# QuantEcon/dynamic_factor_models

Hardware: NVIDIA H100
Metric: EM iters/sec (N=200,r=8,T=500) (higher is better)
Workload: dtype f64

## Files before the change

dynamic_factor_models_b200/csrc/dfm_api.cu:

```cuda
#include "../../include/dfm_b200.h"
#include "dfm_common.cuh"
#include "dfm_kernels_np.cuh"
#include "dfm_kernels_em.cuh"
#include "dfm_kernels_emb.cuh"
#include "dfm_kernels_fused.cuh"
#include "dfm_kernels_fused2.cuh"
#include "dfm_kernels_als_masked.cuh"
#include "dfm_kernels_rep.cuh"
#include "dfm_kernels_inst.cuh"
#include <algorithm>
#include <new>
#include <thread>
#include <vector>
#ifndef DFM_EMU
#include <dlfcn.h>
#endif

#ifdef DFM_EMU
typedef int cudaError_t;
enum { cudaSuccess = 0 };
enum cudaMemcpyKind { cudaMemcpyHostToDevice, cudaMemcpyDeviceToHost, cudaMemcpyDeviceToDevice };
static inline cudaError_t cudaMalloc(void** p, size_t n) { *p = malloc(n ? n : 1); return *p ? 0 : 2; }
static inline cudaError_t cudaFree(void* p) { free(p); return 0; }
static inline cudaError_t cudaMemcpyAsync(void* d, const void* s, size_t n, cudaMemcpyKind, cudaStream_t) { memcpy(d, s, n); return 0; }
// ... 164 lines not shown
    cudaOccupancyMaxActiveBlocksPerMultiprocessor(&occ, k_em_fused<RT>, 128, smem);
    if (occ < 1) occ = 1;
    grid = std::min(B, h->nsm * occ);
  } else grid = std::min(B, h->nsm * 8);
#endif
  double* scr = arena->get<double>((size_t)std::min(B, h->nsm * 8) * T * FUSED_SCR(RT));
  if (dry) return DFM_OK;
  FusedArgs a2 = fa; a2.scratch = scr;
  L(k_em_fused<RT>, grid, 1, 128, smem, a2);
  (void)scratch_out;
  return DFM_OK;
}

struct EmbPlan {
  bool on; int ncb, ntE, nsE, nper, ntM, tsM, tper;
  double *Bpart, *qpart, *Spart, *sxxpart, *Cpart; int* counters;
  size_t smE, smM;
};
static EmbPlan emb_plan(int T, int N, int r, int batch, int nsm) {
  EmbPlan e{};
  e.on = r <= 32 && !getenv("DFM_NO_EMB");
  if (!e.on) return e;
  e.ncb = (r + 7) / 8;
  const int target = 2 * nsm;
  e.ntE = (T + EMB_TILE - 1) / EMB_TILE;
  int want = (target + e.ntE * batch - 1) / (e.ntE * batch);
  int ns = std::max((N + EMB_MAXSPLIT - 1) / EMB_MAXSPLIT, std::min(want, (N + 31) / 32));
  e.nper = (((N + ns - 1) / ns) + 3) & ~3;
  e.nsE = (N + e.nper - 1) / e.nper;
  e.ntM = (N + EMB_TILE - 1) / EMB_TILE;
  want = (target + e.ntM * batch - 1) / (e.ntM * batch);
  int ts = std::max(1, std::min(want, (T + 31) / 32));
  e.tper = (((T + ts - 1) / ts) + 3) & ~3;
  e.tsM = (T + e.tper - 1) / e.tper;
  if ((long long)e.nsE * batch > 65535 || (long long)e.tsM * batch > 65535) { e.on = false; return e; }
  e.smE = ((size_t)e.ncb * 8 * emb_pad(e.nper) + e.nper + 48) * 8;
  e.smM = ((size_t)2 * r * r + (size_t)2 * EMB_TILE * (r + 1) + 96) * 8;
  return e;
}
template <int NCB>
static int emb_launch_E(dfm_handle* h, const EmbPlan& e, const double* x, const double* dW, const double* dR, const double* dlogR, int T, int N,
                        int r, int batch, double* dBt, double* dqt, double* dslr, int* dnt, EmState* st) {
  DFM_SET_SMEM(k_emb_contract<NCB>, e.smE);
  L(k_emb_contract<NCB>, e.ntE, e.nsE * batch, 256, e.smE, x, dW, dR, dlogR, T, N, r, e.nsE, e.nper, batch, e.Bpart, e.qpart, e.counters,
    dBt, dqt, dslr, dnt, st);
  return DFM_OK;
}
template <int NCB>
static int emb_launch_M(dfm_handle* h, const EmbPlan& e, const double* x, const double* dFs, const double* dSff, int T, int N, int r, int batch,
                        double* dL, double* dR, double* dW, double* dlogR, EmState* st) {
  DFM_SET_SMEM(k_emb_mstep<NCB>, e.smM);
  L(k_emb_mstep<NCB>, e.ntM, e.tsM * batch, 256, e.smM, x, dFs, dSff, T, N, r, e.tsM, e.tper, batch, e.Spart, e.sxxpart,
    e.counters + (size_t)batch * e.ntE, dL, dR, dW, dlogR, e.Cpart, st);
  return DFM_OK;
}

static int run_em_general(dfm_handle* h, const double* x, const dfm_em_opts* o, double* dL, double* dR, double* dA, double* dQ, double* dP0,
                          double* dAn, double* dQn, double* dW, double* dlogR, double* dC, double* dBt, double* dqt, double* dslr, int* dnt,
                          double* dCt, double* dzp, double* dzf, double* dPp, double* dPf, double* dFs, double* dPsF, double* dSff, double* dll,
                          EmState* st, int* dit, int* dstat, int* active, int ntC, int nblkC, size_t smFS, int stgT, int want_psf, double* dxch, const EmbPlan& emb) {
  int T = o->T, N = o->N, r = o->r, p = o->p, batch = o->batch, mi = o->max_iter;
  int np = r * (r + 1) / 2;
  int* dsrc = dnt + (size_t)batch * T;
  int ntFS = (batch <= 2 * h->nsm) ? 512 : 256;
  if (getenv("DFM_FS_THREADS")) ntFS = atoi(getenv("DFM_FS_THREADS"));
  int ncl = 1;
  if (dxch && !getenv("DFM_NO_CLUSTER")) { if (batch * 8 <= h->nsm) ncl = 8; else if (batch * 4 <= h->nsm) ncl = 4; else if (batch * 2 <= h->nsm) ncl = 2; }
  if (getenv("DFM_CLUSTER")) ncl = std::max(1, std::min(8, atoi(getenv("DFM_CLUSTER"))));
  L(k_em_state_init, batch, 1, 1, 0, st);
  L(k_em_scan, N, batch, 64, 0, x, dL, T, N, r, st);
  L(k_em_prep, batch, 1, 128, 0, dL, dR, N, r, p, dW, dlogR, dC, dA, dAn, dQ, dQn, st, mi, 0, emb.on ? 1 : 0);
  if (emb.on) {
    L(k_emb_cinit, emb.ntM, batch, 256, 0, dL, dW, N, r, emb.Cpart, st);
    L(k_emb_close, batch, 1, 256, 0, N, r, p, emb.ntM, emb.Cpart, dC, dA, dAn, dQ, dQn, st, mi, 0);
  }
  int n_missing = batch;
  if (emb.on) {
    L(k_em_count_missing, 1, 1, 128, 48 * 8, st, batch, active);
    CK(cudaMemcpyAsync(&n_missing, active, sizeof(int), cudaMemcpyDeviceToHost, h->stream));
    CK(cudaStreamSynchronize(h->stream));
    CK(cudaMemsetAsync(emb.counters, 0, sizeof(int) * (size_t)batch * (emb.ntE + emb.ntM), h->stream));
  }
  const bool any_missing = n_missing > 0, any_bal = emb.on ? (n_missing < batch) : true;
  const int emb_on = emb.on ? 1 : 0;
  int h_active = batch;
  for (int it = 0; it < mi && h_active > 0; ++it) {
    if (any_missing) L(k_em_contract, nblkC, batch, ntC, ((size_t)(np + r) * ntC + 8) * 8, x, dL, dW, dR, dlogR, dC, T, N, r, dBt, dqt, dslr, dnt, dCt, st);
    if (any_bal) {
      if (!emb.on) L(k_em_contract_bal, (T + 31) / 32, batch, 256, 8 * 32 * 3 * 8, x, dW, dR, dlogR, T, N, r, dBt, dqt, dslr, dnt, st);
      else switch (emb.ncb) {
        case 1: emb_launch_E<1>(h, emb, x, dW, dR, dlogR, T, N, r, batch, dBt, dqt, dslr, dnt, st); break;
        case 2: emb_launch_E<2>(h, emb, x, dW, dR, dlogR, T, N, r, batch, dBt, dqt, dslr, dnt, st); break;
        case 3: emb_launch_E<3>(h, emb, x, dW, dR, dlogR, T, N, r, batch, dBt, dqt, dslr, dnt, st); break;
        default: emb_launch_E<4>(h, emb, x, dW, dR, dlogR, T, N, r, batch, dBt, dqt, dslr, dnt, st); break;
      }
    }
#ifndef DFM_EMU
    if (ncl > 1) {
      PROF_BEGIN("k_em_filter_smooth");
      cudaLaunchConfig_t cfg = {};
      cfg.gridDim = dim3((unsigned)(batch * ncl)); cfg.blockDim = dim3((unsigned)ntFS); cfg.dynamicSmemBytes = smFS; cfg.stream = h->stream;
      cudaLaunchAttribute at[1];
      at[0].id = cudaLaunchAttributeClusterDimension; at[0].val.clusterDim.x = (unsigned)ncl; at[0].val.clusterDim.y = 1; at[0].val.clusterDim.z = 1;
      cfg.attrs = at; cfg.numAttrs = 1;
      cudaError_t ce = cudaLaunchKernelEx(&cfg, k_em_filter_smooth, (const double*)dA, (const double*)dQ, (const double*)dP0, (const double*)dC,
                            (const double*)dBt, (const double*)dqt, (const double*)dslr, (const int*)dnt, (const double*)dCt, T, r, p, dzp, dzf,
                            dPp, dPf, dFs, dPsF, dSff, dAn, dQn, dll, mi, o->tol, st, dsrc, stgT, want_psf, dxch);
      PROF_END(); h->launches++;
      if (ce != cudaSuccess) {
        (void)cudaGetLastError();
        ncl = 1;
        L(k_em_filter_smooth, batch, 1, ntFS, smFS, dA, dQ, dP0, dC, dBt, dqt, dslr, dnt, dCt, T, r, p, dzp, dzf, dPp, dPf,
          dFs, dPsF, dSff, dAn, dQn, dll, mi, o->tol, st, dsrc, stgT, want_psf, (double*)nullptr);
      }
    } else
#endif
    L(k_em_filter_smooth, batch, 1, ntFS, smFS, dA, dQ, dP0, dC, dBt, dqt, dslr, dnt, dCt, T, r, p, dzp, dzf, dPp, dPf,
      dFs, dPsF, dSff, dAn, dQn, dll, mi, o->tol, st, dsrc, stgT, want_psf, (double*)nullptr);
    if (any_missing || !emb.on) L(k_em_mstep_series, N, batch, 64, (size_t)(2 * np + r + 8) * 8, x, dFs, dPsF, dSff, T, N, r, dL, dR, st, emb_on);
    if (any_bal && emb.on) {
      switch (emb.ncb) {
        case 1: emb_launch_M<1>(h, emb, x, dFs, dSff, T, N, r, batch, dL, dR, dW, dlogR, st); break;
        case 2: emb_launch_M<2>(h, emb, x, dFs, dSff, T, N, r, batch, dL, dR, dW, dlogR, st); break;
        case 3: emb_launch_M<3>(h, emb, x, dFs, dSff, T, N, r, batch, dL, dR, dW, dlogR, st); break;
        default: emb_launch_M<4>(h, emb, x, dFs, dSff, T, N, r, batch, dL, dR, dW, dlogR, st); break;
      }
      L(k_emb_close, batch, 1, 256, 0, N, r, p, emb.ntM, emb.Cpart, dC, dA, dAn, dQ, dQn, st, mi, 1);
    }
    if (any_missing || !emb.on) L(k_em_prep, batch, 1, 128, 0, dL, dR, N, r, p, dW, dlogR, dC, dA, dAn, dQ, dQn, st, mi, 1, emb_on);
    if (o->tol > 0 && ((it & 3) == 3)) {
      L(k_em_count_active, 1, 1, 128, 48 * 8, st, batch, active);
      CK(cudaMemcpyAsync(&h_active, active, sizeof(int), cudaMemcpyDeviceToHost, h->stream));
      CK(cudaStreamSynchronize(h->stream));
    }
  }
  L(k_em_collect, batch, 1, 1, 0, st, dit, dstat);
  return DFM_OK;
}

template <int RT>
static int launch_fused2(dfm_handle* h, const FusedArgs& fa, int B, int T, int N, Arena* arena, bool dry) {
  size_t smem = fused2_smem_doubles<RT>(T, N) * 8;
  int grid = std::min(B, h->nsm * 8);
  double* scr = arena->get<double>((size_t)std::min(B, h->nsm * 8) * T * FUSED_SCR(RT));
  if (dry) return DFM_OK;
#ifndef DFM_EMU
  DFM_SET_SMEM(k_em_fused2<RT>, smem);
  int occ = 1;
  cudaOccupancyMaxActiveBlocksPerMultiprocessor(&occ, k_em_fused2<RT>, 256, smem);
  if (occ < 1) occ = 1;
  grid = std::min(B, h->nsm * occ);
#endif
  FusedArgs a2 = fa; a2.scratch = scr;
  CUtensorMap tm; int rc_ = make_panel_tmap(h, fa.X, T, (long long)B * N, &tm); if (rc_) return rc_;
  L(k_em_fused2<RT>, grid, 1, 256, smem, a2, tm);
  return DFM_OK;
}

template <int RT>
static int launch_als_fused2(dfm_handle* h, const AlsFusedArgs& fa, int B, int T, int N) {
  size_t smem = als_fused2_smem_doubles<RT>(T, N) * 8;
  int grid = std::min(B, h->nsm * 8);
#ifndef DFM_EMU
  DFM_SET_SMEM(k_als_fused2<RT>, smem);
  int occ = 1;
  cudaOccupancyMaxActiveBlocksPerMultiprocessor(&occ, k_als_fused2<RT>, 256, smem);
  if (occ < 1) occ = 1;
  grid = std::min(B, h->nsm * occ);
#endif
  CUtensorMap tm; int rc_ = make_panel_tmap(h, fa.Xs, T, (long long)B * N, &tm); if (rc_) return rc_;
  L(k_als_fused2<RT>, grid, 1, 256, smem, fa, tm);
  return DFM_OK;
}
template <int RT>
static int launch_als_masked(dfm_handle* h, const AlsMaskedArgs& fa, int B, int T, int N) {
  size_t smem = als_masked_smem_doubles<RT>(T, N) * 8;
  int grid = std::min(B, h->nsm * 2);
#ifndef DFM_EMU
  DFM_SET_SMEM(k_als_masked<RT>, smem);
  int occ = 1;
  cudaOccupancyMaxActiveBlocksPerMultiprocessor(&occ, k_als_masked<RT>, 256, smem);
  if (occ < 1) occ = 1;
  grid = std::min(B, h->nsm * occ);
#endif
  L(k_als_masked<RT>, grid, 1, 256, smem, fa);
  return DFM_OK;
}
static bool als_masked_shape_ok(int T, int N, int r) {
  if (r < 1 || r > 8) return false;
  return ((size_t)r * (T | 1) + (size_t)r * (N | 1) + 5 * (size_t)r * r + 48) * 8 <= 100 * 1024;
}
static bool als_fused2_shape_ok(int T, int N, int r) {
  if (r < 1 || r > 8 || T < 4 || (T & 1)) return false;
  return ((size_t)FZ * pad4mod16(T) + (size_t)r * pad4mod16(N) + (size_t)N + 4 * (size_t)r * r + 2 * r + 48 +
          2 * F2_NCW * 72 + (size_t)F2_S * F2_STG + 32) * 8 <= 113 * 1024;
}

template <int RT> static int fused2_capacity_t(int nsm, int T, int N) {
#ifdef DFM_EMU
  (void)nsm; (void)T; (void)N; return 4;
#else
  size_t smem = fused2_smem_doubles<RT>(T, N) * 8;
  DFM_SET_SMEM(k_em_fused2<RT>, smem);
  int occ = 1;
  cudaOccupancyMaxActiveBlocksPerMultiprocessor(&occ, k_em_fused2<RT>, 256, smem);
  return nsm * (occ < 1 ? 1 : occ);
#endif
}
static int fused2_capacity(int nsm, int r, int T, int N) {
  switch (r) {
#define DFM_CASEC(RT) case RT: return fused2_capacity_t<RT>(nsm, T, N);
    DFM_CASEC(1) DFM_CASEC(2) DFM_CASEC(3) DFM_CASEC(4) DFM_CASEC(5) DFM_CASEC(6) DFM_CASEC(7) DFM_CASEC(8)
#undef DFM_CASEC
  }
  return 1;
}

static bool fused2_shape_ok(int T, int N, int r, int p) {
  if (p != 1 || r < 1 || r > 8 || T < 4 || (T & 1)) return false;
  size_t need = ((size_t)FZ * pad4mod16(T) + (size_t)r * pad4mod16(N) + 3 * (size_t)N + 30 * (size_t)r * r + 2 * (size_t)r +
                 std::max((size_t)97 * r + (size_t)r * r, (size_t)2 * F2_NCW * 72) + (size_t)F2_S * F2_STG + 106) * 8;
  return need <= 113 * 1024;
}

static bool fused_shape_ok(int T, int N, int r, int p) {
  if (p != 1 || r < 1 || r > 8 || T < 3) return false;
  return ((size_t)FZ * pad4mod16(T) + (size_t)r * pad4mod16(N) + 3 * (size_t)N + 31 * (size_t)r * r + 66 * (size_t)r + 128) * 8 <= kMaxSmem;
}

extern "C" {

int dfm_version(void) { return DFM_VERSION; }

const char* dfm_status_string(int s) {
  switch (s) {
    case DFM_OK: return "ok";
    case DFM_ERR_ARG: return "bad argument";
    case DFM_ERR_TOO_FEW_OBS: return "too few observations";
    case DFM_ERR_NOT_PD: return "matrix not positive definite";
    case DFM_ERR_NOT_CONVERGED: return "not converged (max_iter reached)";
    case DFM_ERR_CUDA: return "CUDA error / no device";
    case DFM_ERR_UNSUPPORTED: return "unsupported problem size";
    case DFM_ERR_NCCL: return "NCCL error";
  }
  return "unknown";
}

static void handle_teardown(dfm_handle* h) {
  if (!h) return;
  if (h->stream) cudaStreamSynchronize(h->stream);
  if (h->ws) cudaFree(h->ws);
  if (h->own_stream && h->stream) cudaStreamDestroy(h->stream);
#ifndef DFM_EMU
  if (h->copy_stream) { cudaStreamSynchronize(h->copy_stream); cudaStreamDestroy(h->copy_stream); }
  if (h->pinned_one) cudaFreeHost(h->pinned_one);
  if (h->d2h_stream) { cudaStreamSynchronize(h->d2h_stream); cudaStreamDestroy(h->d2h_stream); }
  if (h->done_host) cudaFreeHost(h->done_host);
  if (h->prof) for (auto& r : *h->prof) { cudaEventDestroy(r.e0); cudaEventDestroy(r.e1); }
#endif
  delete h->prof;
  delete h;
}

int dfm_create_on_stream(int device, void* cuda_stream, dfm_handle** out) {
  if (!out) return DFM_ERR_ARG;
  *out = nullptr;
  int ndev = 0;
  if (cudaGetDeviceCount(&ndev) != cudaSuccess || ndev <= 0 || device < 0 || device >= ndev) return DFM_ERR_CUDA;
  if (cudaSetDevice(device) != cudaSuccess) return DFM_ERR_CUDA;
  dfm_handle* h = new (std::nothrow) dfm_handle();
  if (!h) return DFM_ERR_CUDA;
  h->device = device; h->ws = nullptr; h->ws_bytes = 0; h->launches = 0; h->err[0] = 0;
  h->nsm = 132;
  h->profile = 0; h->prof = new std::vector<ProfRec>();
  h->stream = nullptr; h->own_stream = false;
  h->copy_stream = nullptr; h->pinned_one = nullptr; h->d2h_stream = nullptr; h->done_host = nullptr; h->done_dev = nullptr; h->done_cap = 0;
#ifndef DFM_EMU
  if (cudaDeviceGetAttribute(&h->nsm, cudaDevAttrMultiProcessorCount, device) != cudaSuccess || h->nsm <= 0) { handle_teardown(h); return DFM_ERR_CUDA; }
  if (cudaStreamCreateWithFlags(&h->copy_stream, cudaStreamNonBlocking) != cudaSuccess) { h->copy_stream = nullptr; handle_teardown(h); return DFM_ERR_CUDA; }
  if (cudaStreamCreateWithFlags(&h->d2h_stream, cudaStreamNonBlocking) != cudaSuccess) { h->d2h_stream = nullptr; handle_teardown(h); return DFM_ERR_CUDA; }
  if (cudaHostAlloc((void**)&h->pinned_one, sizeof(int), cudaHostAllocDefault) != cudaSuccess) { h->pinned_one = nullptr; handle_teardown(h); return DFM_ERR_CUDA; }
  *h->pinned_one = 1;
#endif
  if (cuda_stream) { h->stream = (cudaStream_t)cuda_stream; h->own_stream = false; }
  else { if (cudaStreamCreate(&h->stream) != cudaSuccess) { h->stream = nullptr; handle_teardown(h); return DFM_ERR_CUDA; } h->own_stream = true; }
  DFM_SET_SMEM(k_em_filter_smooth, kMaxSmem); DFM_SET_SMEM(k_als_factor, kMaxSmem); DFM_SET_SMEM(k_em_contract, kMaxSmem);
  DFM_SET_SMEM(k_lyapunov, kMaxSmem); DFM_SET_SMEM(k_var, kMaxSmem); DFM_SET_SMEM(k_pca_finish, kMaxSmem);
  DFM_SET_SMEM(k_jacobi, kMaxSmem); DFM_SET_SMEM(k_subspace_eig, kMaxSmem); DFM_SET_SMEM(k_loading, kMaxSmem); DFM_SET_SMEM(k_als_lambda, kMaxSmem);
  if (cudaGetLastError() != cudaSuccess) { handle_teardown(h); return DFM_ERR_CUDA; }
  *out = h;
  return DFM_OK;
}
int dfm_create(int device, dfm_handle** out) { return dfm_create_on_stream(device, nullptr, out); }

int dfm_destroy(dfm_handle* h) {
  if (!h) return DFM_ERR_ARG;
  cudaSetDevice(h->device);
  handle_teardown(h);
  return DFM_OK;
}
int dfm_sync(dfm_handle* h) { if (!h) return DFM_ERR_ARG; CK(cudaStreamSynchronize(h->stream)); return DFM_OK; }
long long dfm_launch_count(const dfm_handle* h) { return h ? h->launches : -1; }
const char* dfm_last_error(const dfm_handle* h) { return h ? h->err : "null handle"; }

int dfm_debug_fs_prof(dfm_handle* h, int on, double* out) {
#ifndef DFM_EMU
// ... 893 lines not shown
```

dynamic_factor_models_b200/csrc/dfm_kernels_fused.cuh:

```cuda
#pragma once
#include "dfm_common.cuh"

namespace dfm {

#define FZ 8
#define ZI(t_, i_) ((i_) * Tp + (t_))
#define LI(n_, c_) ((c_) * Np + (n_))
__host__ __device__ inline int pad4mod16(int x) { return x + ((4 - x % 16) + 16) % 16; }

#define DFM_PH 32
struct FusedArgs {
  const double* X;
  double* Lam;
  double* R;
  double* A;
  double* Q;
  const double* P0;
  double* Fs;
  double* PsF;
  double* loglik;
  int* iters; int* status;
  double* scratch;
  int B, T, N, max_iter;
  double tol;
  const int* ready; int ready_chunk;
  int* done;
  double* P0out;
  int p0_steps;
  int stagger;
  long long* phase_cycles;
};
#ifdef DFM_EMU
#define DFM_TICK(k_) ((void)0)
#else
#define DFM_TICK(k_) do { if (a.phase_cycles && threadIdx.x == 0) { long long now_ = clock64(); a.phase_cycles[(size_t)blockIdx.x * DFM_PH + (k_)] += now_ - tick_; tick_ = now_; } } while (0)
#endif
#define FUSED_SCR(R_) (5 * (R_) * (R_) + 1)

__device__ __forceinline__ double w_max(double v) {
#ifndef DFM_EMU
  for (int o = 16; o > 0; o >>= 1) v = fmax(v, __shfl_xor_sync(0xffffffffu, v, o));
#endif
  return v;
}

#ifdef DFM_EMU
#define DFM_HELPER inline
#else
#define DFM_HELPER __device__ __noinline__
#endif
template <int R>
DFM_HELPER void w_gemm(double* C, const double* A, bool ta, const double* B, bool tb) {
#ifndef DFM_EMU
  if (R == 8) {
    const int lane = threadIdx.x & 31, lr = lane >> 2, lc = lane & 3;
    double d0 = 0.0, d1 = 0.0;
#pragma unroll
    for (int kc = 0; kc < 2; ++kc) {
      const int kk = 4 * kc + lc;
      const double av = ta ? A[kk * 8 + lr] : A[lr * 8 + kk];
      const double bv = tb ? B[lr * 8 + kk] : B[kk * 8 + lr];
      asm volatile("mma.sync.aligned.m8n8k4.row.col.f64.f64.f64.f64 {%0,%1}, {%2}, {%3}, {%0,%1};\n"
                   : "+d"(d0), "+d"(d1) : "d"(av), "d"(bv));
    }
    C[lr * 8 + 2 * lc] = d0; C[lr * 8 + 2 * lc + 1] = d1;
    __syncwarp();
    return;
  }
#endif
  for (int e = DFM_LANE; e < R * R; e += DFM_WSZ) {
    int i = e / R, j = e % R;
    double s = 0.0;
#pragma unroll
    for (int l = 0; l < R; ++l) s += (ta ? A[l * R + i] : A[i * R + l]) * (tb ? B[j * R + l] : B[l * R + j]);
    C[e] = s;
  }
  DFM_WSYNC();
}
template <int R>
DFM_HELPER void w_sym(double* A) {
#ifndef DFM_EMU
  if (R == 8) {
    const int lane = threadIdx.x & 31, i = lane >> 2, j0 = 2 * (lane & 3);
    const double v0 = 0.5 * (A[i * 8 + j0] + A[j0 * 8 + i]), v1 = 0.5 * (A[i * 8 + j0 + 1] + A[(j0 + 1) * 8 + i]);
    __syncwarp();
    A[i * 8 + j0] = v0; A[i * 8 + j0 + 1] = v1;
    __syncwarp();
    return;
  }
#endif
  for (int e = DFM_LANE; e < R * R; e += DFM_WSZ) {
    int i = e / R, j = e % R;
    if (i > j) { double v = 0.5 * (A[i * R + j] + A[j * R + i]); A[i * R + j] = v; A[j * R + i] = v; }
  }
  DFM_WSYNC();
}
template <int R>
DFM_HELPER double w_inv(double* Ai, const double* A, double* tmp, int* bad) {
#ifndef DFM_EMU
  if (R == 8) {
    const int lane = threadIdx.x & 31, i = lane >> 2, q = lane & 3, j0 = 2 * q;
    double x0 = A[i * 8 + j0], x1 = A[i * 8 + j0 + 1];
    double pp = 1.0;
#pragma unroll
    for (int p = 0; p < 8; ++p) {
      const double sel = (p & 1) ? x1 : x0;
      double piv = __shfl_sync(0xffffffffu, sel, p * 4 + (p >> 1));
      const double rp0 = __shfl_sync(0xffffffffu, x0, p * 4 + q);
      const double rp1 = __shfl_sync(0xffffffffu, x1, p * 4 + q);
      const double cp = __shfl_sync(0xffffffffu, sel, (lane & ~3) + (p >> 1));
      if (!(piv > 0.0)) { *bad = 1; piv = 1.0; }
      pp *= piv;
      const double d = 1.0 / piv, cd = cp * d;
      const bool ip = (i == p);
      x0 = ip ? ((j0 == p) ? d : rp0 * d) : ((j0 == p) ? -cd : x0 - cd * rp0);
      x1 = ip ? ((j0 + 1 == p) ? d : rp1 * d) : ((j0 + 1 == p) ? -cd : x1 - cd * rp1);
    }
    Ai[i * 8 + j0] = x0; Ai[i * 8 + j0 + 1] = x1;
    __syncwarp();
    (void)tmp;
    return log(pp);
  }
#endif
  for (int e = DFM_LANE; e < R * R; e += DFM_WSZ) Ai[e] = A[e];
  DFM_WSYNC();
  double pp = 1.0;
  for (int p = 0; p < R; ++p) {
    for (int e = DFM_LANE; e < R; e += DFM_WSZ) { tmp[e] = Ai[p * R + e]; tmp[R + e] = Ai[e * R + p]; }
    DFM_WSYNC();
    double piv = tmp[p];
    if (!(piv > 0.0)) { *bad = 1; piv = 1.0; }
    pp *= piv;
    double d = 1.0 / piv;
    for (int e = DFM_LANE; e < R * R; e += DFM_WSZ) {
      int i = e / R, j = e % R;
      double v;
      if (i == p && j == p) v = d;
      else if (i == p) v = tmp[j] * d;
      else if (j == p) v = -tmp[R + i] * d;
      else v = Ai[e] - tmp[R + i] * tmp[j] * d;
      Ai[e] = v;
    }
    DFM_WSYNC();
  }
  return log(pp);
}

__device__ __forceinline__ int blk_chunk_len(int n, int ng) {
  int Lc = (n + ng - 1) / ng;
  if (Lc > 1 && !(Lc & 1)) Lc += 1;
  return Lc;
}

template <int R>
__device__ __forceinline__ void w_matpow(double* pw, const double* Cf, int ex0, double* base, double* pw2) {
  for (int e = DFM_LANE; e < R * R; e += DFM_WSZ) { int i = e / R, j = e % R; pw[e] = (i == j) ? 1.0 : 0.0; base[e] = Cf[e]; }
  DFM_WSYNC();
  for (int ex = ex0; ex > 0; ex >>= 1) {
    if (ex & 1) { w_gemm<R>(pw2, pw, false, base, false); for (int e = DFM_LANE; e < R * R; e += DFM_WSZ) pw[e] = pw2[e]; DFM_WSYNC(); }
    if (ex > 1) { w_gemm<R>(pw2, base, false, base, false); for (int e = DFM_LANE; e < R * R; e += DFM_WSZ) base[e] = pw2[e]; DFM_WSYNC(); }
  }
}

template <int R>
__device__ __forceinline__ void blk_recur(double* Z, int Tp, const double* Cf, double* pw, double* pw2, double* bnd, int t0, int n, int dir, int nthr,
                                          long long* prof = nullptr, bool pw_ready = false, const double* pl1 = nullptr, const double* pl2 = nullptr,
                                          const double* pl3 = nullptr, const double* pl4 = nullptr) {
  if (n <= 0) return;
  const int ng = nthr / 8;
#ifndef DFM_EMU
#define BLK_SYNC() asm volatile("bar.sync 2, %0;" ::"r"(nthr) : "memory")
#else
#define BLK_SYNC() ((void)0)
#endif
#ifndef DFM_EMU
  long long pt_ = prof ? clock64() : 0;
#define BLK_PROF(k_) do { if (prof && threadIdx.x == 0) { long long now_ = clock64(); prof[k_] += now_ - pt_; pt_ = now_; } } while (0)
#else
#define BLK_PROF(k_) ((void)0)
#endif
  const int Lc = blk_chunk_len(n, ng);
  const int nch = (n + Lc - 1) / Lc;
// ... 579 lines not shown
```

dynamic_factor_models_b200/csrc/dfm_kernels_fused2.cuh:

```cuda
#pragma once
#include <algorithm>
#include "dfm_kernels_fused.cuh"
#ifdef DFM_EMU
struct CUtensorMap { char opaque[128]; };
#define DFM_GRID_CONSTANT
#else
#include <cuda.h>
#define DFM_GRID_CONSTANT __grid_constant__
#endif

namespace dfm {

#ifndef F2_SBS
#define F2_SBS 1
#endif
#ifndef F2_S
#define F2_S (4 / F2_SBS)
#endif
#define F2_STG (F2_SBS * 8 * F2_TS)
#ifndef F2_TC
#define F2_TC 132
#endif
#define F2_TS F2_TC
#define F2_NCW 6
#define F2_GPARTS_S 4
#define F2_GPARTS ((R == 8) ? (F2_NCW + 1) : F2_GPARTS_S)
#define F2_NRB (((F2_TC + 7) / 8 + F2_NCW - 1) / F2_NCW)
#define F2_NKC (((F2_TC + 3) / 4 + F2_NCW - 1) / F2_NCW)
static_assert(F2_TC % 16 == 4 || F2_TC % 16 == 12, "ring pitch must be 4 or 12 mod 16");
static_assert(F2_TC <= 256 && (F2_TC * 64) % 128 == 0, "TMA box / stage alignment");
#define F2_NEXS(R_) ((F2_S * F2_STG - 4 * (R_) * (R_)) / FUSED_SCR(R_))
#define F2_RTAIL(R_) (F2_S * F2_STG - 4 * (R_) * (R_))

#ifndef DFM_EMU
__device__ __forceinline__ uint32_t f2_smem_u32(const void* p) { return (uint32_t)__cvta_generic_to_shared(p); }
__device__ __forceinline__ void f2_mbar_init(uint64_t* bar, int cnt) { asm volatile("mbarrier.init.shared::cta.b64 [%0], %1;" ::"r"(f2_smem_u32(bar)), "r"(cnt)); }
__device__ __forceinline__ void f2_mbar_expect(uint64_t* bar, uint32_t bytes) { asm volatile("mbarrier.arrive.expect_tx.shared::cta.b64 _, [%0], %1;" ::"r"(f2_smem_u32(bar)), "r"(bytes) : "memory"); }
__device__ __forceinline__ void f2_mbar_arrive(uint64_t* bar) { asm volatile("mbarrier.arrive.shared::cta.b64 _, [%0];" ::"r"(f2_smem_u32(bar)) : "memory"); }
__device__ __forceinline__ void f2_mbar_wait(uint64_t* bar, uint32_t phase) {
  asm volatile("{\n.reg .pred p;\nWAIT_%=:\nmbarrier.try_wait.parity.shared::cta.b64 p, [%0], %1;\n@p bra DONE_%=;\nbra WAIT_%=;\nDONE_%=:\n}" ::"r"(f2_smem_u32(bar)), "r"(phase) : "memory");
}
__device__ __forceinline__ void f2_tma_2d(void* dst, const CUtensorMap* tmap, int x, int y, uint64_t* bar) {
  asm volatile("cp.async.bulk.tensor.2d.shared::cluster.global.mbarrier::complete_tx::bytes [%0], [%1, {%2, %3}], [%4];"
               ::"r"(f2_smem_u32(dst)), "l"(reinterpret_cast<uint64_t>(tmap)), "r"(x), "r"(y), "r"(f2_smem_u32(bar)) : "memory");
}
#endif


#ifndef DFM_EMU
struct F2Ring {
  double* ring; uint64_t* full; uint64_t* empty;
  int rs; uint32_t rph; bool wrap;
  __device__ __forceinline__ void advance() { if (++rs == F2_S) { rs = 0; rph ^= 1; wrap = true; } }
  __device__ __forceinline__ void skip(long long n) { for (long long q = 0; q < n; ++q) advance(); }
};

__device__ __forceinline__ void f2_produce(F2Ring& rg, const CUtensorMap* tmap, int row0, int T, int N, bool c_outer) {
  const int lane = threadIdx.x & 31;
  const int nsb = (N + 8 * F2_SBS - 1) / (8 * F2_SBS), nck = (T + F2_TC - 1) / F2_TC;
  const int n_out = c_outer ? nck : nsb, n_in = c_outer ? nsb : nck;
  for (int o = 0; o < n_out; ++o)
    for (int i = 0; i < n_in; ++i) {
      const int c = c_outer ? o : i, sb = c_outer ? i : o;
      if (rg.wrap) f2_mbar_wait(&rg.empty[rg.rs], rg.rph ^ 1);
      if (lane == 0) {
        f2_mbar_expect(&rg.full[rg.rs], (uint32_t)(F2_STG * 8));
        f2_tma_2d(rg.ring + (size_t)rg.rs * F2_STG, tmap, c * F2_TC, row0 + sb * 8 * F2_SBS, &rg.full[rg.rs]);
      }
      __syncwarp();
      rg.advance();
    }
}

template <int R>
__device__ __forceinline__ double f2_consume_E(F2Ring& rg, int cw, int T, int N, int Tp, int Np, double* Z, const double* Lam,
                                               const double* rinv) {
  const int lane = threadIdx.x & 31, lr = lane >> 2, lc = lane & 3;
  const int nsg = (N + 8 * F2_SBS - 1) / (8 * F2_SBS), nck = (T + F2_TC - 1) / F2_TC;
  double qacc = 0.0;
  for (int c = 0; c < nck; ++c) {
    const int len = (T - c * F2_TC < F2_TC) ? T - c * F2_TC : F2_TC;
    double d[F2_NRB][2][2];
#pragma unroll
    for (int j = 0; j < F2_NRB; ++j) { d[j][0][0] = 0.0; d[j][0][1] = 0.0; d[j][1][0] = 0.0; d[j][1][1] = 0.0; }
    for (int sg = 0; sg < nsg; ++sg) {
      f2_mbar_wait(&rg.full[rg.rs], rg.rph);
      const double* stage = rg.ring + (size_t)rg.rs * F2_STG;
#pragma unroll
      for (int sub = 0; sub < F2_SBS; ++sub) {
        const double* tile = stage + (size_t)sub * 8 * F2_TS;
        const int sb = sg * F2_SBS + sub;
        double rn[2], lm[2], av[2][F2_NRB];
#pragma unroll
        for (int kc = 0; kc < 2; ++kc) {
          const int n = sb * 8 + kc * 4 + lc;
          const bool nok = n < N;
          rn[kc] = nok ? (rinv ? rinv[n] : 1.0) : 0.0;
          lm[kc] = (nok && lr < R) ? Lam[LI(n, lr)] : 0.0;
          const double* trow = tile + (kc * 4 + lc) * F2_TS + lr;
#pragma unroll
          for (int j = 0; j < F2_NRB; ++j) {
            const int t0 = (cw + j * F2_NCW) * 8;
            av[kc][j] = (nok && t0 + lr < len) ? trow[t0] : 0.0;
          }
        }
#pragma unroll
        for (int kc = 0; kc < 2; ++kc)
#pragma unroll
          for (int j = 0; j < F2_NRB; ++j) {
            const double ar = av[kc][j] * rn[kc];
            qacc += av[kc][j] * ar;
            asm volatile("mma.sync.aligned.m8n8k4.row.col.f64.f64.f64.f64 {%0,%1}, {%2}, {%3}, {%0,%1};\n"
                         : "+d"(d[j][kc][0]), "+d"(d[j][kc][1]) : "d"(ar), "d"(lm[kc]));
          }
      }
      __syncwarp();
      if (lane == 0) f2_mbar_arrive(&rg.empty[rg.rs]);
      rg.advance();
    }
#pragma unroll
    for (int j = 0; j < F2_NRB; ++j) {
      const int tl = (cw + j * F2_NCW) * 8 + lr;
      if (tl < len) { const int t = c * F2_TC + tl; Z[ZI(t, 2 * lc)] = d[j][0][0] + d[j][1][0]; Z[ZI(t, 2 * lc + 1)] = d[j][0][1] + d[j][1][1]; }
    }
  }
  return qacc;
}

template <int R>
__device__ __forceinline__ void f2_consume_M(F2Ring& rg, int cw, int T, int N, int Tp, int Np, const double* Z, double* Lam,
                                             double* sxx, double* part) {
  const int lane = threadIdx.x & 31, lr = lane >> 2, lc = lane & 3;
  const int nsg = (N + 8 * F2_SBS - 1) / (8 * F2_SBS), nck = (T + F2_TC - 1) / F2_TC;
  double d[F2_SBS][F2_NKC][2], s2[F2_SBS];
#pragma unroll
  for (int sub = 0; sub < F2_SBS; ++sub) {
    s2[sub] = 0.0;
#pragma unroll
    for (int j = 0; j < F2_NKC; ++j) { d[sub][j][0] = 0.0; d[sub][j][1] = 0.0; }
  }
  for (int sg = 0; sg < nsg; ++sg)
    for (int c = 0; c < nck; ++c) {
      f2_mbar_wait(&rg.full[rg.rs], rg.rph);
      const double* stage = rg.ring + (size_t)rg.rs * F2_STG;
      const int len = (T - c * F2_TC < F2_TC) ? T - c * F2_TC : F2_TC;
      const double* zc = Z + (size_t)lr * Tp + c * F2_TC + lc;
      double bv[F2_NKC];
#pragma unroll
      for (int j = 0; j < F2_NKC; ++j) { const int t0 = (cw + j * F2_NCW) * 4; bv[j] = (t0 + lc < len) ? zc[t0] : 0.0; }
#pragma unroll
      for (int sub = 0; sub < F2_SBS; ++sub) {
        const bool nok = (sg * F2_SBS + sub) * 8 + lr < N;
        const double* trow = stage + (size_t)sub * 8 * F2_TS + lr * F2_TS + lc;
        double av[F2_NKC];
#pragma unroll
        for (int j = 0; j < F2_NKC; ++j) { const int t0 = (cw + j * F2_NCW) * 4; av[j] = (nok && t0 + lc < len) ? trow[t0] : 0.0; }
#pragma unroll
        for (int j = 0; j < F2_NKC; ++j) {
          s2[sub] += av[j] * av[j];
          asm volatile("mma.sync.aligned.m8n8k4.row.col.f64.f64.f64.f64 {%0,%1}, {%2}, {%3}, {%0,%1};\n"
                       : "+d"(d[sub][j][0]), "+d"(d[sub][j][1]) : "d"(av[j]), "d"(bv[j]));
        }
      }
      __syncwarp();
      if (lane == 0) f2_mbar_arrive(&rg.empty[rg.rs]);
      rg.advance();
      if (c == nck - 1) {
#pragma unroll
        for (int sub = 0; sub < F2_SBS; ++sub) {
          const int sb = sg * F2_SBS + sub;
          double sq = s2[sub];
          sq += __shfl_xor_sync(0xffffffffu, sq, 1); sq += __shfl_xor_sync(0xffffffffu, sq, 2);
          double* pb = part + (size_t)(sb & 1) * F2_NCW * 72 + cw * 72;
          double t0_ = 0.0, t1_ = 0.0;
#pragma unroll
          for (int j = 0; j < F2_NKC; ++j) { t0_ += d[sub][j][0]; t1_ += d[sub][j][1]; d[sub][j][0] = 0.0; d[sub][j][1] = 0.0; }
          pb[2 * lane] = t0_; pb[2 * lane + 1] = t1_;
          if (lc == 0) pb[64 + lr] = sq;
          asm volatile("bar.sync 1, %0;" ::"n"(F2_NCW * 32) : "memory");
          const int ct = cw * 32 + lane;
          if (ct < 72) {
            const double* pp_ = part + (size_t)(sb & 1) * F2_NCW * 72 + ct;
            double tot_ = 0.0;
#pragma unroll
            for (int w_ = 0; w_ < F2_NCW; ++w_) tot_ += pp_[w_ * 72];
            if (ct < 64) {
              const int l_ = ct >> 1, h_ = ct & 1, row = l_ >> 2, col = 2 * (l_ & 3) + h_, n = sb * 8 + row;
              if (n < N && col < R) Lam[LI(n, col)] = tot_;
            } else { const int n = sb * 8 + (ct - 64); if (n < N) sxx[n] = tot_; }
          }
          s2[sub] = 0.0;
        }
      }
    }
}
#endif

#ifdef DFM_EMU
#define F2_ROLE_T0() ((void)0)
#define F2_ROLE_T1(k_) ((void)0)
#define F2_SUB(k_) ((void)0)
#define F2_SUBP(k_) nullptr
#define F2_PSYNC() ((void)0)
#define F2_PTID 0
#define F2_PNT 1
#define F2_PNT_GPU ((F2_NCW + 1) * 32)
#else
#define F2_ROLE_T0() long long role_t0_ = a.phase_cycles ? clock64() : 0
#define F2_ROLE_T1(k_) do { if (a.phase_cycles && DFM_LANE == 0) a.phase_cycles[(size_t)blockIdx.x * DFM_PH + (k_)] += clock64() - role_t0_; } while (0)
#define F2_SUB(k_) do { if (a.phase_cycles && threadIdx.x == 0) { long long now_ = clock64(); a.phase_cycles[(size_t)blockIdx.x * DFM_PH + (k_)] += now_ - sub_; sub_ = now_; } } while (0)
#define F2_SUBP(k_) (a.phase_cycles ? a.phase_cycles + (size_t)blockIdx.x * DFM_PH + (k_) : nullptr)
#define F2_PNT_GPU ((F2_NCW + 1) * 32)
#define F2_PSYNC() asm volatile("bar.sync 2, %0;" ::"n"(F2_PNT_GPU) : "memory")
#define F2_PTID ((int)threadIdx.x)
#define F2_PNT F2_PNT_GPU
#endif
#ifdef DFM_EMU
#define DFM_FUSED2_BOUNDS
#else
#define DFM_FUSED2_BOUNDS __launch_bounds__(256, 2)
#endif
template <int R>
__global__ void DFM_FUSED2_BOUNDS k_em_fused2(FusedArgs a, const DFM_GRID_CONSTANT CUtensorMap tmap) {
  DFM_SMEM(sm);
  constexpr int RR = R * R, NP = R * (R + 1) / 2;
  const int T = a.T, N = a.N;
  const int Tp = pad4mod16(T), Np = pad4mod16(N);
  double* Z = sm;
  double* Lam = Z + (size_t)FZ * Tp;
  double* rinv = Lam + (size_t)R * Np;
  double* Rv = rinv + N;
  double* sxx = Rv + N;
  double* mats = sxx + N;
  double* M = mats;            double* Q = M + RR;        double* C = Q + RR;        double* Pp = C + RR;
  double* Pi = Pp + RR;        double* Pf = Pi + RR;      double* Wm = Pf + RR;      double* G = Wm + RR;
  double* Phi = G + RR;        double* Jm = Phi + RR;     double* Pn = Jm + RR;      double* T1 = Pn + RR;
  double* T2 = T1 + RR;        double* Ps = T2 + RR;      double* Psn = Ps + RR;     double* SPall = Psn + RR;
  double* SP00 = SPall + RR;   double* SPff2 = SP00 + RR; double* SP11 = SPff2 + RR; double* Sm = SP11 + RR;
  double* S11m = Sm + RR;      double* Pfinf = S11m + RR; double* Phinf = Pfinf + RR; double* Jinf = Phinf + RR;
  double* Winf = Jinf + RR;    double* Ppinf = Winf + RR; double* IJM = Ppinf + RR;  double* Pfprev = IJM + RR;
  double* tmp = Pfprev + RR;
  double* red = tmp + 2 * R;
  double* scal = red + 40;
  int* ctl = (int*)(scal + 8);
  double* bnd = scal + 16;
  double* part = bnd;
  double* ring = bnd + (((size_t)97 * R + RR > 2 * F2_NCW * 72) ? (size_t)97 * R + RR : 2 * F2_NCW * 72);
#ifndef DFM_EMU
  ring += ((128u - (f2_smem_u32(ring) & 127u)) & 127u) / 8;
#endif
  double* gscr = a.scratch + (size_t)DFM_BX * T * FUSED_SCR(R);
#define GSC(t_) (gscr + (size_t)(t_) * FUSED_SCR(R))
#define SCRP(t_) (((t_) < F2_NEXS(R)) ? (ring + (size_t)(t_) * FUSED_SCR(R)) : (gscr + (size_t)(t_) * FUSED_SCR(R)))
#define GPS(t_) (gscr + (size_t)(t_) * FUSED_SCR(R) + 4 * RR)
#ifndef DFM_EMU
  __shared__ uint64_t fullb[F2_S], emptyb[F2_S];
  if (threadIdx.x == 0) { for (int s_ = 0; s_ < F2_S; ++s_) { f2_mbar_init(&fullb[s_], 1); f2_mbar_init(&emptyb[s_], F2_NCW); } }
  asm volatile("fence.mbarrier_init.release.cluster;" ::: "memory");
  __syncthreads();
  F2Ring rg; rg.ring = ring; rg.full = fullb; rg.empty = emptyb; rg.rs = 0; rg.rph = 0; rg.wrap = false;
#endif
  const double eps = 1e-14;
#ifndef DFM_EMU
  long long tick_ = clock64();
#endif

#ifndef DFM_EMU
  if (a.stagger > 0 && blockIdx.x >= gridDim.x / 2) { long long t0_ = clock64(); while (clock64() - t0_ < a.stagger) __nanosleep(500); }
#endif
  for (int b = DFM_BX; b < a.B; b += DFM_GX) {
    const double* X = a.X + (size_t)b * T * N;
#ifndef DFM_EMU
    if (a.ready) {
      if (threadIdx.x == 0) {
        const int* f_ = a.ready + b / a.ready_chunk; int v_ = 0;
        for (;;) { asm volatile("ld.acquire.sys.global.s32 %0, [%1];" : "=r"(v_) : "l"(f_) : "memory"); if (v_) break; __nanosleep(256); }
      }
      __syncthreads();
// ... 76 lines not shown
        int* bad = &ctl[2];
        for (int e = DFM_LANE; e < RR; e += DFM_WSZ) { int i = e / R, j = e % R; Pp[e] = a.P0[(size_t)b * RR + i + R * j]; }
        DFM_WSYNC();
        int nE = T, frozen_at = -1, t = 0;
#ifndef DFM_EMU
        long long c0_ = clock64();
#endif
        while (t < T) {
          double ldp = w_inv<R>(Pi, Pp, tmp, bad);
          for (int e = DFM_LANE; e < RR; e += DFM_WSZ) Wm[e] = Pi[e] + C[e];
          DFM_WSYNC();
          double ldw = w_inv<R>(Pf, Wm, tmp, bad);
          w_gemm<R>(G, Pf, false, Pi, false);
          w_gemm<R>(Phi, G, false, M, false);
          if (t >= 1) { w_gemm<R>(T1, Pfprev, false, M, true); w_gemm<R>(Jm, T1, false, Pi, false); }
          w_gemm<R>(T1, M, false, Pf, false);
          w_gemm<R>(Pn, T1, false, M, true);
          for (int e = DFM_LANE; e < RR; e += DFM_WSZ) Pn[e] += Q[e];
          DFM_WSYNC();
          w_sym<R>(Pn);
          double* s_ = GSC(t);
          double dmax = 0.0, pmax = 0.0;
          for (int e = DFM_LANE; e < RR; e += DFM_WSZ) {
            s_[e] = Pf[e]; s_[RR + e] = Phi[e]; s_[3 * RR + e] = Wm[e];
            if (t >= 1) GSC(t - 1)[2 * RR + e] = Jm[e];
            dmax = fmax(dmax, fabs(Pn[e] - Pp[e])); pmax = fmax(pmax, fabs(Pp[e]));
            Pfprev[e] = Pf[e];
          }
          if (DFM_LANE == 0) s_[5 * RR] = ldp + ldw;
          dmax = w_max(dmax); pmax = w_max(pmax);
          DFM_WSYNC();
          if (frozen_at >= 0 && t == frozen_at + 1) {
            nE = t + 1;
            for (int e = DFM_LANE; e < RR; e += DFM_WSZ) { Pfinf[e] = Pf[e]; Phinf[e] = Phi[e]; Winf[e] = Wm[e]; }
            if (DFM_LANE == 0) scal[1] = ldp + ldw;
            DFM_WSYNC();
            w_gemm<R>(T1, Pf, false, M, true);
            w_gemm<R>(Jinf, T1, false, Pi, false);
            break;
          }
          if (frozen_at < 0 && dmax <= eps * pmax) frozen_at = t;
          for (int e = DFM_LANE; e < RR; e += DFM_WSZ) Pp[e] = Pn[e];
          DFM_WSYNC();
          ++t;
        }
        const int frozen = nE < T;
        if (DFM_LANE == 0) { ctl[0] = nE; ctl[3] = frozen; }
#ifndef DFM_EMU
        if (a.phase_cycles && DFM_LANE == 0) a.phase_cycles[(size_t)blockIdx.x * DFM_PH + 12] += clock64() - c0_;
#endif
        if (frozen) {
          w_gemm<R>(IJM, Jinf, false, M, false);
          for (int e = DFM_LANE; e < RR; e += DFM_WSZ) { int i = e / R, j = e % R; IJM[e] = ((i == j) ? 1.0 : 0.0) - IJM[e]; }
          DFM_WSYNC();
          const int n3 = T - (nE > 0 ? nE : 1), n5 = (T - 2) - (nE - 1) + 1;
          if (n3 > 0) {
            w_matpow<R>(Phi, Phinf, blk_chunk_len(n3, F2_PNT_GPU / 8), T1, T2);
            w_gemm<R>(Pp, Phi, false, Phi, false); w_gemm<R>(Pi, Pp, false, Pp, false);
            w_gemm<R>(Pf, Pi, false, Pi, false);   w_gemm<R>(Jm, Pf, false, Pf, false);
          }
          if (n5 > 0) {
            w_matpow<R>(Pn, Jinf, blk_chunk_len(n5, F2_PNT_GPU / 8), T1, T2);
            double* gl_ = GSC(T - 1);
            w_gemm<R>(T1, Pn, false, Pn, false);
            for (int e = DFM_LANE; e < RR; e += DFM_WSZ) gl_[e] = T1[e];
            w_gemm<R>(T2, T1, false, T1, false);
            for (int e = DFM_LANE; e < RR; e += DFM_WSZ) gl_[RR + e] = T2[e];
            w_gemm<R>(T1, T2, false, T2, false);
            for (int e = DFM_LANE; e < RR; e += DFM_WSZ) gl_[2 * RR + e] = T1[e];
            w_gemm<R>(T2, T1, false, T1, false);
            for (int e = DFM_LANE; e < RR; e += DFM_WSZ) gl_[3 * RR + e] = T2[e];
            DFM_WSYNC();
          }
        }
        DFM_WSYNC();
      };
      auto chain_bwd = [&]() {
        const int nE = ctl[0], frozen = ctl[3];
        int t;
#ifndef DFM_EMU
        long long c1_ = a.phase_cycles ? clock64() : 0;
#endif
        for (int e = DFM_LANE; e < RR; e += DFM_WSZ) {
          double v = frozen ? Pfinf[e] : (GSC(T - 1))[e];
          Psn[e] = v; SPall[e] = v; SPff2[e] = v; SP00[e] = 0.0; SP11[e] = 0.0;
          GPS(T - 1)[e] = v;
        }
        DFM_WSYNC();
        const int lo = frozen ? nE - 1 : T;
        int tb = -1;
        t = T - 2;
        while (t >= 0) {
          const double* pf_t = (t < nE) ? GSC(t) : Pfinf;
          const double* j_t = (t < nE - 1) ? GSC(t) + 2 * RR : Jinf;
          w_gemm<R>(T1, M, false, pf_t, false);
          w_gemm<R>(T2, T1, false, M, true);
          for (int e = DFM_LANE; e < RR; e += DFM_WSZ) T2[e] = Psn[e] - (T2[e] + Q[e]);
          DFM_WSYNC();
          w_sym<R>(T2);
          w_gemm<R>(T1, j_t, false, T2, false);
          w_gemm<R>(Ps, T1, false, j_t, true);
          for (int e = DFM_LANE; e < RR; e += DFM_WSZ) Ps[e] += pf_t[e];
          DFM_WSYNC();
          w_sym<R>(Ps);
          w_gemm<R>(T1, Psn, false, j_t, true);
          double dmax = 0.0, pmax = 0.0;
          for (int e = DFM_LANE; e < RR; e += DFM_WSZ) {
            SP11[e] += T1[e]; SPall[e] += Ps[e]; SP00[e] += Ps[e];
            if (t >= 1) SPff2[e] += Ps[e];
            GPS(t)[e] = Ps[e];
            dmax = fmax(dmax, fabs(Ps[e] - Psn[e])); pmax = fmax(pmax, fabs(Ps[e]));
          }
          dmax = w_max(dmax); pmax = w_max(pmax);
          DFM_WSYNC();
          bool conv = frozen && t > lo && dmax <= eps * pmax;
          for (int e = DFM_LANE; e < RR; e += DFM_WSZ) Psn[e] = Ps[e];
          DFM_WSYNC();
          if (conv) {
            tb = t;
            double cnt = (double)(t - lo);
            w_gemm<R>(T1, Ps, false, Jinf, true);
            for (int e = DFM_LANE; e < RR; e += DFM_WSZ) {
              SPall[e] += cnt * Ps[e]; SP00[e] += cnt * Ps[e];
              SPff2[e] += ((lo >= 1) ? cnt : cnt - 1.0) * Ps[e];
              SP11[e] += cnt * T1[e];
              Ppinf[e] = Ps[e];
            }
            DFM_WSYNC();
            t = lo - 1;
          } else --t;
        }
        if (DFM_LANE == 0) ctl[1] = tb;
#ifndef DFM_EMU
        if (a.phase_cycles && DFM_LANE == 0) a.phase_cycles[(size_t)blockIdx.x * DFM_PH + 13] += clock64() - c1_;
#endif
#ifdef DFM_EMU
        if (getenv("DFM_DEBUG_CHAIN")) printf("[chain] b=%d it=%d nE=%d frozen=%d tb=%d (T=%d)\n", b, it, nE, frozen, tb, T);
#endif
        DFM_WSYNC();
      };
      double qacc = 0.0;
#ifdef DFM_EMU
      for (int t = 0; t < T; ++t) {
        for (int c = 0; c < FZ; ++c) Z[ZI(t, c)] = 0.0;
        for (int n = 0; n < N; ++n) {
          double x = X[(size_t)n * T + t], xr = x * rinv[n];
          qacc += x * xr;
          for (int c = 0; c < R; ++c) Z[ZI(t, c)] += xr * Lam[LI(n, c)];
        }
      }
#else
      {
        const long long nitems = (long long)((N + 8 * F2_SBS - 1) / (8 * F2_SBS)) * ((T + F2_TC - 1) / F2_TC);
        F2_ROLE_T0();
        if (DFM_WARP == 0) { f2_produce(rg, &tmap, b * N, T, N, true); F2_ROLE_T1(14); }
        else if (DFM_WARP <= F2_NCW) { qacc += f2_consume_E<R>(rg, DFM_WARP - 1, T, N, Tp, Np, Z, Lam, rinv); if (DFM_WARP == 1) F2_ROLE_T1(15); }
        else {
          rg.skip(nitems);
          chain_fwd();
        }
      }
#endif
#ifdef DFM_EMU
      chain_fwd();
      chain_bwd();
#endif
      DFM_SYNC();
      DFM_TICK(2);
      const int nE = ctl[0], frozen = ctl[3];
      DFM_TICK(3);
#ifndef DFM_EMU
      long long sub_ = a.phase_cycles ? clock64() : 0;
#endif
#ifndef DFM_EMU
      if (DFM_WARP == F2_NCW + 1) chain_bwd();
      else
#endif
      {
      {
        const int ncp = (nE < F2_NEXS(R)) ? nE : F2_NEXS(R);
        for (int e = F2_PTID; e < ncp * FUSED_SCR(R); e += F2_PNT) ring[e] = gscr[e];
        if (frozen) for (int e = F2_PTID; e < 4 * RR; e += F2_PNT) ring[F2_RTAIL(R) + e] = GSC(T - 1)[e];
      }
      for (int t = nE + F2_PTID; t < T; t += F2_PNT) {
        double bb[R], u[R];
#pragma unroll
        for (int j = 0; j < R; ++j) bb[j] = Z[ZI(t, j)];
#pragma unroll
        for (int i = 0; i < R; ++i) { double s = 0.0;
#pragma unroll
          for (int j = 0; j < R; ++j) s += Pfinf[i * R + j] * bb[j]; u[i] = s; }
#pragma unroll
        for (int i = 0; i < R; ++i) Z[ZI(t, i)] = u[i];
      }
      F2_PSYNC();
      F2_SUB(20);
      if (DFM_WARP == 0) {
        for (int t = 0; t < nE; ++t) {
          const double* s_ = SCRP(t);
          for (int i = DFM_LANE; i < R; i += DFM_WSZ) {
            double s = 0.0;
            for (int j = 0; j < R; ++j) s += s_[i * R + j] * Z[ZI(t, j)];
            if (t >= 1) for (int j = 0; j < R; ++j) s += s_[RR + i * R + j] * Z[ZI(t - 1, j)];
            tmp[i] = s;
          }
          DFM_WSYNC();
          for (int i = DFM_LANE; i < R; i += DFM_WSZ) Z[ZI(t, i)] = tmp[i];
          DFM_WSYNC();
        }
      }
      F2_PSYNC();
      F2_SUB(21);
      if (frozen) blk_recur<R>(Z, Tp, Phinf, Phi, Pi, bnd, (nE > 0 ? nE : 1), T - (nE > 0 ? nE : 1), +1, F2_PNT_GPU, F2_SUBP(22), true, Pp, Pi, Pf, Jm);
      DFM_TICK(4);
      double llp = -0.5 * qacc;
      const bool gram = frozen && nE >= 1 && nE < T;
      const bool split = gram && 2 * nE * R <= (97 * R + RR) - (F2_GPARTS + 1) * RR;
      const int tex = gram ? (split ? 0 : nE) : T;
      if (gram) {
        double* gp = bnd;
#ifndef DFM_EMU
        if (R == 8) {
          const int lr = DFM_LANE >> 2, lc = DFM_LANE & 3;
          const double* zr = Z + (size_t)lr * Tp;
          double g0 = 0.0, g1 = 0.0, h0 = 0.0, h1 = 0.0;
          for (int t0 = nE + 4 * DFM_WARP; t0 < T; t0 += 8 * (F2_NCW + 1)) {
            const int ta = t0 + lc, tb_ = t0 + 4 * (F2_NCW + 1) + lc;
            const double va = (ta < T) ? zr[ta] : 0.0, vb = (tb_ < T) ? zr[tb_] : 0.0;
            asm volatile("mma.sync.aligned.m8n8k4.row.col.f64.f64.f64.f64 {%0,%1}, {%2}, {%3}, {%0,%1};\n" : "+d"(g0), "+d"(g1) : "d"(va), "d"(va));
            asm volatile("mma.sync.aligned.m8n8k4.row.col.f64.f64.f64.f64 {%0,%1}, {%2}, {%3}, {%0,%1};\n" : "+d"(h0), "+d"(h1) : "d"(vb), "d"(vb));
          }
          gp[DFM_WARP * 64 + 2 * DFM_LANE] = g0 + h0; gp[DFM_WARP * 64 + 2 * DFM_LANE + 1] = g1 + h1;
        } else
#endif
        {
          const int nfz = T - nE, q4 = (nfz + F2_GPARTS_S - 1) / F2_GPARTS_S;
          for (int e = F2_PTID; e < F2_GPARTS * RR; e += F2_PNT) {
            const int q = e / RR, ee = e % RR, i = ee / R, jj = ee % R;
            double s0_ = 0.0, s1_ = 0.0;
            if (q < F2_GPARTS_S) {
              const int lo = nE + q * q4, hi = (lo + q4 < T) ? lo + q4 : T;
              int t = lo;
              for (; t + 1 < hi; t += 2) { s0_ += Z[ZI(t, i)] * Z[ZI(t, jj)]; s1_ += Z[ZI(t + 1, i)] * Z[ZI(t + 1, jj)]; }
              if (t < hi) s0_ += Z[ZI(t, i)] * Z[ZI(t, jj)];
            }
            gp[e] = s0_ + s1_;
          }
        }
        if (split) {
          double* zd = gp + (F2_GPARTS + 1) * RR;
          for (int e = F2_PTID; e < nE * R; e += F2_PNT) {
            const int t = e / R, i = e % R;
            double s_ = 0.0;
            if (t >= 1) {
#pragma unroll
              for (int j = 0; j < R; ++j) s_ += M[i * R + j] * Z[ZI(t - 1, j)];
            }
            zd[2 * e] = s_; zd[2 * e + 1] = Z[ZI(t, i)] - s_;
          }
        }
        if (DFM_WARP == 0) {
          for (int e = DFM_LANE; e < RR; e += DFM_WSZ) Wm[e] = Winf[e] - C[e];
          DFM_WSYNC();
          w_gemm<R>(G, Wm, false, M, false);
          w_gemm<R>(gp + F2_GPARTS * RR, M, true, G, false);
        }
        F2_PSYNC();
        for (int e = F2_PTID; e < RR; e += F2_PNT) {
          const int i = e / R, jj = e % R;
          double gf = 0.0;
#pragma unroll
          for (int q = 0; q < F2_GPARTS; ++q) gf += gp[q * RR + e];
          const double gs = gf + Z[ZI(nE - 1, i)] * Z[ZI(nE - 1, jj)] - Z[ZI(T - 1, i)] * Z[ZI(T - 1, jj)];
          llp += -0.5 * (gp[F2_GPARTS * RR + e] * gs - Winf[e] * gf);
        }
        if (F2_PTID == 0) llp += -0.5 * (double)(T - nE) * ((double)N * 1.8378770664093454835606594728112 + scal[0] + scal[1]);
        if (split) {
          const double* zd = gp + (F2_GPARTS + 1) * RR;
          for (int e = F2_PTID; e < nE * R; e += F2_PNT) {
            const int t = e / R, i = e % R;
            const double* Wt = SCRP(t) + 3 * RR;
            const double* zt = zd + 2 * (size_t)t * R;
            double cz = 0.0, g = 0.0;
#pragma unroll
            for (int j = 0; j < R; ++j) { cz += C[i * R + j] * zt[2 * j]; g += Wt[i * R + j] * zt[2 * j + 1]; }
            const double zpi = zt[2 * i], di = zt[2 * i + 1];
            llp += 0.5 * (zpi * cz + 2.0 * zpi * g + g * di);
            if (i == 0) llp += -0.5 * ((double)N * 1.8378770664093454835606594728112 + scal[0] + (SCRP(t))[5 * RR]);
          }
        }
      }
      for (int t = F2_PTID; t < tex; t += F2_PNT) {
        const double* Wt = (t < nE) ? SCRP(t) + 3 * RR : Winf;
        double ldt = (t < nE) ? (SCRP(t))[5 * RR] : scal[1];
        double zp[R], d[R];
#pragma unroll
        for (int i = 0; i < R; ++i) { double s = 0.0; if (t >= 1) {
#pragma unroll
            for (int j = 0; j < R; ++j) s += M[i * R + j] * Z[ZI(t - 1, j)]; }
          zp[i] = s; d[i] = Z[ZI(t, i)] - s; }
        double quad = 0.0;
#pragma unroll
        for (int i = 0; i < R; ++i) {
          double cz = 0.0, g = 0.0;
#pragma unroll
          for (int j = 0; j < R; ++j) { cz += C[i * R + j] * zp[j]; g += Wt[i * R + j] * d[j]; }
          quad -= zp[i] * cz + 2.0 * zp[i] * g + g * d[i];
        }
        llp += -0.5 * ((double)N * 1.8378770664093454835606594728112 + scal[0] + ldt + quad);
// ... 323 lines not shown
```

Baseline: 1.208 million.

## Reverse E-step panel traversal to reuse L2-resident data when panels exceed L2

Adds a reversed, series-outer traversal of the X panel in the fused EM E-step. The TMA producer walks series blocks and time chunks backward, and a new consumer keeps per-chunk accumulators in registers across all series blocks. The aim is to hit in L2 on data the previous phase touched last, rather than refetching from HBM. It is turned on only when the total panel footprint across the grid exceeds the L2 size, and an environment variable can override that. The cost is more accumulator registers per consumer warp, which could lower occupancy or cause spills.

```diff
diff --git a/dynamic_factor_models_b200/csrc/dfm_api.cu b/dynamic_factor_models_b200/csrc/dfm_api.cu
--- a/dynamic_factor_models_b200/csrc/dfm_api.cu
+++ b/dynamic_factor_models_b200/csrc/dfm_api.cu
@@ -340,6 +340,11 @@
   grid = std::min(B, h->nsm * occ);
 #endif
   FusedArgs a2 = fa; a2.scratch = scr;
+#ifndef DFM_EMU
+  int l2_ = 0; cudaDeviceGetAttribute(&l2_, cudaDevAttrL2CacheSize, h->device);
+  a2.e_rev = (long long)grid * T * N * 8 > (long long)l2_;
+  if (const char* ev_ = getenv("DFM_FUSED_EREV")) a2.e_rev = atoi(ev_) != 0;
+#endif
   CUtensorMap tm; int rc_ = make_panel_tmap(h, fa.X, T, (long long)B * N, &tm); if (rc_) return rc_;
   L(k_em_fused2<RT>, grid, 1, 256, smem, a2, tm);
   return DFM_OK;
diff --git a/dynamic_factor_models_b200/csrc/dfm_kernels_fused.cuh b/dynamic_factor_models_b200/csrc/dfm_kernels_fused.cuh
--- a/dynamic_factor_models_b200/csrc/dfm_kernels_fused.cuh
+++ b/dynamic_factor_models_b200/csrc/dfm_kernels_fused.cuh
@@ -28,6 +28,7 @@
   double* P0out;
   int p0_steps;
   int stagger;
+  int e_rev;
   long long* phase_cycles;
 };
 #ifdef DFM_EMU
diff --git a/dynamic_factor_models_b200/csrc/dfm_kernels_fused2.cuh b/dynamic_factor_models_b200/csrc/dfm_kernels_fused2.cuh
--- a/dynamic_factor_models_b200/csrc/dfm_kernels_fused2.cuh
+++ b/dynamic_factor_models_b200/csrc/dfm_kernels_fused2.cuh
@@ -55,12 +55,13 @@
   __device__ __forceinline__ void skip(long long n) { for (long long q = 0; q < n; ++q) advance(); }
 };
 
-__device__ __forceinline__ void f2_produce(F2Ring& rg, const CUtensorMap* tmap, int row0, int T, int N, bool c_outer) {
+__device__ __forceinline__ void f2_produce(F2Ring& rg, const CUtensorMap* tmap, int row0, int T, int N, bool c_outer, bool rev = false) {
   const int lane = threadIdx.x & 31;
   const int nsb = (N + 8 * F2_SBS - 1) / (8 * F2_SBS), nck = (T + F2_TC - 1) / F2_TC;
   const int n_out = c_outer ? nck : nsb, n_in = c_outer ? nsb : nck;
-  for (int o = 0; o < n_out; ++o)
-    for (int i = 0; i < n_in; ++i) {
+  for (int o_ = 0; o_ < n_out; ++o_)
+    for (int i_ = 0; i_ < n_in; ++i_) {
+      const int o = rev ? n_out - 1 - o_ : o_, i = rev ? n_in - 1 - i_ : i_;
       const int c = c_outer ? o : i, sb = c_outer ? i : o;
       if (rg.wrap) f2_mbar_wait(&rg.empty[rg.rs], rg.rph ^ 1);
       if (lane == 0) {
@@ -124,6 +125,69 @@
       if (tl < len) { const int t = c * F2_TC + tl; Z[ZI(t, 2 * lc)] = d[j][0][0] + d[j][1][0]; Z[ZI(t, 2 * lc + 1)] = d[j][0][1] + d[j][1][1]; }
     }
   }
+  return qacc;
+}
+
+template <int R>
+__device__ __forceinline__ double f2_consume_Er(F2Ring& rg, int cw, int T, int N, int Tp, int Np, double* Z, const double* Lam,
+                                                const double* rinv) {
+  static_assert(F2_SBS == 1, "one series block per stage");
+  const int lane = threadIdx.x & 31, lr = lane >> 2, lc = lane & 3;
+  const int nsb = (N + 7) / 8, nck = (T + F2_TC - 1) / F2_TC;
+  double qacc = 0.0;
+  double d[F2_S][F2_NRB][2];
+#pragma unroll
+  for (int c = 0; c < F2_S; ++c)
+#pragma unroll
+    for (int j = 0; j < F2_NRB; ++j) { d[c][j][0] = 0.0; d[c][j][1] = 0.0; }
+  for (int sb = nsb - 1; sb >= 0; --sb) {
+    double rn[2], lm[2];
+    bool nok[2];
+#pragma unroll
+    for (int kc = 0; kc < 2; ++kc) {
+      const int n = sb * 8 + kc * 4 + lc;
+      nok[kc] = n < N;
+      rn[kc] = nok[kc] ? rinv[n] : 0.0;
+      lm[kc] = (nok[kc] && lr < R) ? Lam[LI(n, lr)] : 0.0;
+    }
+#pragma unroll
+    for (int c = F2_S - 1; c >= 0; --c) {
+      if (c < nck) {
+        f2_mbar_wait(&rg.full[rg.rs], rg.rph);
+        const int len = (T - c * F2_TC < F2_TC) ? T - c * F2_TC : F2_TC;
+        const double* tile = rg.ring + (size_t)rg.rs * F2_STG;
+        double av[2][F2_NRB];
+#pragma unroll
+        for (int kc = 0; kc < 2; ++kc) {
+          const double* trow = tile + (kc * 4 + lc) * F2_TS + lr;
+#pragma unroll
+          for (int j = 0; j < F2_NRB; ++j) {
+            const int t0 = (cw + j * F2_NCW) * 8;
+            av[kc][j] = (nok[kc] && t0 + lr < len) ? trow[t0] : 0.0;
+          }
+        }
+#pragma unroll
+        for (int kc = 0; kc < 2; ++kc)
+#pragma unroll
+          for (int j = 0; j < F2_NRB; ++j) {
+            const double ar = av[kc][j] * rn[kc];
+            qacc += av[kc][j] * ar;
+            asm volatile("mma.sync.aligned.m8n8k4.row.col.f64.f64.f64.f64 {%0,%1}, {%2}, {%3}, {%0,%1};\n"
+                         : "+d"(d[c][j][0]), "+d"(d[c][j][1]) : "d"(ar), "d"(lm[kc]));
+          }
+        __syncwarp();
+        if (lane == 0) f2_mbar_arrive(&rg.empty[rg.rs]);
+        rg.advance();
+      }
+    }
+  }
+#pragma unroll
+  for (int c = 0; c < F2_S; ++c)
+#pragma unroll
+    for (int j = 0; j < F2_NRB; ++j) {
+      const int tl = (cw + j * F2_NCW) * 8 + lr, len = (T - c * F2_TC < F2_TC) ? T - c * F2_TC : F2_TC;
+      if (tl < len) { const int t = c * F2_TC + tl; Z[ZI(t, 2 * lc)] = d[c][j][0]; Z[ZI(t, 2 * lc + 1)] = d[c][j][1]; }
+    }
   return qacc;
 }
 
@@ -506,9 +570,13 @@
 #else
       {
         const long long nitems = (long long)((N + 8 * F2_SBS - 1) / (8 * F2_SBS)) * ((T + F2_TC - 1) / F2_TC);
+        const bool erev = a.e_rev && F2_SBS == 1 && T <= F2_S * F2_TC;
         F2_ROLE_T0();
-        if (DFM_WARP == 0) { f2_produce(rg, &tmap, b * N, T, N, true); F2_ROLE_T1(14); }
-        else if (DFM_WARP <= F2_NCW) { qacc += f2_consume_E<R>(rg, DFM_WARP - 1, T, N, Tp, Np, Z, Lam, rinv); if (DFM_WARP == 1) F2_ROLE_T1(15); }
+        if (DFM_WARP == 0) { f2_produce(rg, &tmap, b * N, T, N, !erev, erev); F2_ROLE_T1(14); }
+        else if (DFM_WARP <= F2_NCW) {
+          qacc += erev ? f2_consume_Er<R>(rg, DFM_WARP - 1, T, N, Tp, Np, Z, Lam, rinv) : f2_consume_E<R>(rg, DFM_WARP - 1, T, N, Tp, Np, Z, Lam, rinv);
+          if (DFM_WARP == 1) F2_ROLE_T1(15);
+        }
         else {
           rg.skip(nitems);
           chain_fwd();
```

Measured after the change: 1.249 million, median of 6. 1.03x the previous value.
